# crowsonkb/style_transfer2

Hardware: AMD Instinct MI355X
Metric: style-transfer iters/sec @1024px VGG19 (higher is better)
Workload: dtype f32; 1 GPU; configs[1]: 1024x1024 single image per GPU, VGG19 to conv5_1, content conv4_2 + 5 style layers, adam fp32, 500 iterations per image; jobs=1, parallelism=independent jobs, 1 per GPU, no collective (replicas)

## Files before the change

style_transfer2_amd/csrc/gram.hip:

```cpp
#include "st2_kernels.h"
#include "env.h"
#include "wave_reduce.h"
#include <stdint.h>
#include <stdlib.h>

namespace st2 {

typedef float f32x16 __attribute__((ext_vector_type(16)));

constexpr int GKT = 32;
constexpr int GLD = GKT + 1;

GramPlan gram_plan(int C, int hw)
{
    GramPlan p;
    p.bt = C > 64 ? 128 : 64;
    const int t = (C + p.bt - 1) / p.bt;
    p.tiles = t * (t + 1) / 2;
    const int target128 = (int)env_int("ST2_GRAM_BLOCKS", 512), target64 = (int)env_int("ST2_GRAM_BLOCKS64", 1024);
    int want = p.bt == 128 ? target128 / p.tiles : (target64 + p.tiles - 1) / p.tiles;
    const int max_splits = (hw + 4 * GKT - 1) / (4 * GKT);
    if (want > max_splits) want = max_splits;
    if (want < 1) want = 1;
    int kslab = (hw + want - 1) / want;
    kslab = (kslab + GKT - 1) / GKT * GKT;
    p.kslab = kslab;
    p.splits = (hw + kslab - 1) / kslab;
    p.slab_floats = (size_t)p.splits * C * C;
    return p;
}

GramPlan gram_plan16(int C, int hw)
{
    GramPlan p = gram_plan(C, hw);
    p.kslab = (p.kslab + 63) / 64 * 64;
    p.splits = (hw + p.kslab - 1) / p.kslab;
    p.slab_floats = (size_t)p.splits * C * C;
    return p;
}

template <int BT>
__global__ __launch_bounds__(256) void gram_partial_k(const float* __restrict__ F, float* __restrict__ slabs,
                                                      int C, int hw, int tiles_1d, int kslab, GramRoi roi)
{
    constexpr int T = BT / 64;
    constexpr int ROWS_PER_T = BT / 8;
    __shared__ float As[BT * GLD];
    __shared__ float Bs[BT * GLD];

    const int tid = threadIdx.x, lane = tid & 63, wave = tid >> 6;
    const int wm = wave >> 1, wn = wave & 1;
    const int n_ut = tiles_1d * (tiles_1d + 1) / 2;
    int tile = blockIdx.x % n_ut;
    const int split = blockIdx.x / n_ut;
    int ti = 0;
    while (tile >= tiles_1d - ti) { tile -= tiles_1d - ti; ++ti; }
    const int tj = ti + tile;
    const int i0 = ti * BT, j0 = tj * BT;
    const bool diag = ti == tj;
    const int kbeg = split * kslab;
    const int kend = min(hw, kbeg + kslab);

    const int sk = tid & 31, sr = tid >> 5;
    float ra[ROWS_PER_T], rb[ROWS_PER_T];

    auto load = [&](int k0) {
        const int k = k0 + sk;
        const int ky = k / roi.rw, kx = k - ky * roi.rw;
        const size_t pix = (size_t)(roi.y0 + ky) * roi.pitch + roi.x0 + kx;
#pragma unroll
        for (int it = 0; it < ROWS_PER_T; ++it) {
            const int r = sr + it * 8;
            ra[it] = (i0 + r < C && k < kend) ? F[(size_t)(i0 + r) * roi.plane + pix] : 0.f;
            if (!diag) rb[it] = (j0 + r < C && k < kend) ? F[(size_t)(j0 + r) * roi.plane + pix] : 0.f;
        }
    };
    auto store = [&]() {
#pragma unroll
        for (int it = 0; it < ROWS_PER_T; ++it) {
            const int r = sr + it * 8;
            As[r * GLD + sk] = ra[it];
            if (!diag) Bs[r * GLD + sk] = rb[it];
        }
    };

    f32x16 acc[T][T];
#pragma unroll
    for (int i = 0; i < T; ++i)
#pragma unroll
        for (int j = 0; j < T; ++j)
#pragma unroll
            for (int e = 0; e < 16; ++e) acc[i][j][e] = 0.f;

    const float* bsrc = diag ? As : Bs;
    const int khalf = lane >> 5, l31 = lane & 31;
    const float* a_base = As + (wm * (T * 32) + l31) * GLD + khalf;
    const float* b_base = bsrc + (wn * (T * 32) + l31) * GLD + khalf;

    load(kbeg);
    for (int k0 = kbeg; k0 < kend; k0 += GKT) {
        __syncthreads();
        store();
        __syncthreads();
        if (k0 + GKT < kend) load(k0 + GKT);
#pragma unroll
        for (int ks = 0; ks < GKT / 2; ++ks) {
            float av[T], bv[T];
#pragma unroll
            for (int i = 0; i < T; ++i) av[i] = a_base[i * 32 * GLD + 2 * ks];
#pragma unroll
            for (int j = 0; j < T; ++j) bv[j] = b_base[j * 32 * GLD + 2 * ks];
#pragma unroll
            for (int i = 0; i < T; ++i)
#pragma unroll
                for (int j = 0; j < T; ++j)
                    acc[i][j] = __builtin_amdgcn_mfma_f32_32x32x2f32(av[i], bv[j], acc[i][j], 0, 0, 0);
        }
    }

    float* dst = slabs + (size_t)split * C * C;
#pragma unroll
    for (int i = 0; i < T; ++i)
#pragma unroll
        for (int j = 0; j < T; ++j) {
            const int col = j0 + wn * (T * 32) + j * 32 + l31;
#pragma unroll
            for (int e = 0; e < 16; ++e) {
                const int row = i0 + wm * (T * 32) + i * 32 + (e & 3) + 8 * (e >> 2) + 4 * khalf;
                if (row < C && col < C) dst[(size_t)row * C + col] = acc[i][j][e];
            }
        }
}

typedef __attribute__((address_space(3))) void* gram_lptr_t;
typedef float gf32x4 __attribute__((ext_vector_type(4)));

template <int BT>
__device__ __forceinline__ void gram_partial_dma_body(const float* __restrict__ F, unsigned f_bytes, float* __restrict__ slabs,
                                                      int C, int hw, int tiles_1d, int kslab)
{
    constexpr int T = BT / 64;
    constexpr int IMG = BT * 32;
    constexpr int PIECES = IMG / 256;
    constexpr int PPW = PIECES / 4;
    __shared__ __attribute__((aligned(16))) float smem[2][2][IMG];

    const int tid = threadIdx.x, lane = tid & 63;
    const int wave = __builtin_amdgcn_readfirstlane(tid >> 6);
    const int wm = wave >> 1, wn = wave & 1;
    const int n_ut = tiles_1d * (tiles_1d + 1) / 2;
    int tile = blockIdx.x % n_ut;
    const int split = blockIdx.x / n_ut;
    int ti = 0;
    while (tile >= tiles_1d - ti) { tile -= tiles_1d - ti; ++ti; }
    const int tj = ti + tile;
    const int i0 = ti * BT, j0 = tj * BT;
    const bool diag = ti == tj;
    const int kbeg = split * kslab;
    const int kend = min(hw, kbeg + kslab);
    const int nsteps = (kend - kbeg) / 32;

    const __amdgpu_buffer_rsrc_t rs = __builtin_amdgcn_make_buffer_rsrc((void*)F, 0, f_bytes, 0x00020000);
    unsigned aoff[PPW], boff[PPW];
#pragma unroll
    for (int t = 0; t < PPW; ++t) {
        const int slot = (wave + 4 * t) * 64 + lane;
        const int r = slot >> 3, q = (slot & 7) ^ ((r >> 1) & 7);
        aoff[t] = i0 + r < C ? ((unsigned)(i0 + r) * (unsigned)hw + (unsigned)kbeg + 4u * q) * 4u : 0xffffffffu;
        boff[t] = j0 + r < C ? ((unsigned)(j0 + r) * (unsigned)hw + (unsigned)kbeg + 4u * q) * 4u : 0xffffffffu;
    }
    auto dma = [&](int step, int stage) {
        const unsigned so = (unsigned)step * 128u;
#pragma unroll
        for (int t = 0; t < PPW; ++t) {
            __builtin_amdgcn_raw_ptr_buffer_load_lds(rs, (gram_lptr_t)(smem[stage][0] + (wave + 4 * t) * 256), 16,
                                                     aoff[t] == 0xffffffffu ? aoff[t] : aoff[t] + so, 0, 0, 0);
            if (!diag)
                __builtin_amdgcn_raw_ptr_buffer_load_lds(rs, (gram_lptr_t)(smem[stage][1] + (wave + 4 * t) * 256), 16,
                                                         boff[t] == 0xffffffffu ? boff[t] : boff[t] + so, 0, 0, 0);
        }
    };

    f32x16 acc[T][T];
#pragma unroll
    for (int i = 0; i < T; ++i)
#pragma unroll
        for (int j = 0; j < T; ++j)
#pragma unroll
            for (int e = 0; e < 16; ++e) acc[i][j][e] = 0.f;

    const int l31 = lane & 31;
    const bool hi = lane >= 32;
    int arow[T], brow[T];
#pragma unroll
    for (int i = 0; i < T; ++i) { arow[i] = wm * (T * 32) + i * 32 + l31; brow[i] = wn * (T * 32) + i * 32 + l31; }

    if (nsteps > 0) dma(0, 0);
    for (int st = 0; st < nsteps; ++st) {
        const int cur = st & 1;
        asm volatile("s_waitcnt vmcnt(0)" ::: "memory");
        __syncthreads();
        if (st + 1 < nsteps) dma(st + 1, cur ^ 1);
        const float* As = smem[cur][0];
        const float* Bs = diag ? smem[cur][0] : smem[cur][1];
#pragma unroll
        for (int q = 0; q < 8; ++q) {
            float a0[T], a1[T], b0[T], b1[T];
#pragma unroll
            for (int i = 0; i < T; ++i) {
                const gf32x4 v = *reinterpret_cast<const gf32x4*>(As + (arow[i] * 8 + (q ^ ((arow[i] >> 1) & 7))) * 4);
                a0[i] = hi ? v.y : v.x; a1[i] = hi ? v.w : v.z;
            }
#pragma unroll
            for (int j = 0; j < T; ++j) {
                const gf32x4 v = *reinterpret_cast<const gf32x4*>(Bs + (brow[j] * 8 + (q ^ ((brow[j] >> 1) & 7))) * 4);
                b0[j] = hi ? v.y : v.x; b1[j] = hi ? v.w : v.z;
            }
#pragma unroll
            for (int i = 0; i < T; ++i)
#pragma unroll
                for (int j = 0; j < T; ++j) {
                    acc[i][j] = __builtin_amdgcn_mfma_f32_32x32x2f32(a0[i], b0[j], acc[i][j], 0, 0, 0);
                    acc[i][j] = __builtin_amdgcn_mfma_f32_32x32x2f32(a1[i], b1[j], acc[i][j], 0, 0, 0);
                }
        }
    }

    const int khalf = lane >> 5;
    float* dst = slabs + (size_t)split * C * C;
#pragma unroll
    for (int i = 0; i < T; ++i)
#pragma unroll
        for (int j = 0; j < T; ++j) {
            const int col = j0 + wn * (T * 32) + j * 32 + l31;
#pragma unroll
            for (int e = 0; e < 16; ++e) {
                const int row = i0 + wm * (T * 32) + i * 32 + (e & 3) + 8 * (e >> 2) + 4 * khalf;
                if (row < C && col < C) dst[(size_t)row * C + col] = acc[i][j][e];
            }
        }
}

__global__ __launch_bounds__(256, 2) void gram_partial_dma_128(const float* F, unsigned f_bytes, float* slabs, int C, int hw, int tiles_1d, int kslab)
{ gram_partial_dma_body<128>(F, f_bytes, slabs, C, hw, tiles_1d, kslab); }
__global__ __launch_bounds__(256, 2) void gram_partial_dma_64(const float* F, unsigned f_bytes, float* slabs, int C, int hw, int tiles_1d, int kslab)
{ gram_partial_dma_body<64>(F, f_bytes, slabs, C, hw, tiles_1d, kslab); }

hipError_t launch_gram_partial(const float* F, float* slabs, int C, int hw, const GramPlan& pl, hipStream_t s,
                               const GramRoi* roi_in)
{
    const int t1 = (C + pl.bt - 1) / pl.bt;
    const unsigned grid = (unsigned)(pl.tiles * pl.splits);
    GramRoi roi = roi_in ? *roi_in : GramRoi{0, 0, hw, hw, (size_t)hw};
    if (!roi_in && !env_off("ST2_GRAM_DMA") && hw % 32 == 0 && pl.kslab % 32 == 0 && (reinterpret_cast<uintptr_t>(F) & 15) == 0 &&
        4ull * C * hw < 0xfffffff0ull) {
        const unsigned fb = (unsigned)(4ull * C * hw);
        if (pl.bt == 128) gram_partial_dma_128<<<grid, 256, 0, s>>>(F, fb, slabs, C, hw, t1, pl.kslab);
        else gram_partial_dma_64<<<grid, 256, 0, s>>>(F, fb, slabs, C, hw, t1, pl.kslab);
        return hipGetLastError();
    }
    if (pl.bt == 128) gram_partial_k<128><<<grid, 256, 0, s>>>(F, slabs, C, hw, t1, pl.kslab, roi);
    else gram_partial_k<64><<<grid, 256, 0, s>>>(F, slabs, C, hw, t1, pl.kslab, roi);
    return hipGetLastError();
}

__global__ __launch_bounds__(256) void gram_reduce_k(const float* __restrict__ slabs, const float* __restrict__ target,
                                                     float* __restrict__ out, float* __restrict__ partial,
                                                     int cc, int splits, float n, int C, int out_ld, int bt)
{
    __shared__ float scratch[4];
    float acc[1] = {0.f};
    for (int i = blockIdx.x * 256 + threadIdx.x; i < cc; i += gridDim.x * 256) {
        const int r = i / C, c = i - r * C;
        const int tr = r / bt, tc = c / bt;
        if (tr > tc) continue;
        float sum = 0.f;
        for (int s = 0; s < splits; ++s) sum += slabs[(size_t)s * cc + i];
        float v = sum / n;
        if (target) v -= target[i];
        out[r * out_ld + c] = v;
        acc[0] += v * v;
        if (tr < tc) { out[c * out_ld + r] = v; acc[0] += v * v; }
    }
    block_sum(acc, scratch);
    if (threadIdx.x == 0 && partial) partial[blockIdx.x] = acc[0];
}

__global__ __launch_bounds__(256) void gram_fold_k(const float* __restrict__ slabs, float* __restrict__ folded,
                                                   int cc, int splits, int per_group, int C, int bt)
{
    const int i = blockIdx.x * 256 + threadIdx.x;
    const int g = blockIdx.y;
    if (i >= cc) return;
    if ((i / C) / bt > (i % C) / bt) return;
    const int s0 = g * per_group, s1 = min(splits, s0 + per_group);
    float sum = 0.f;
    for (int s = s0; s < s1; ++s) sum += slabs[(size_t)s * cc + i];
    folded[(size_t)g * cc + i] = sum;
}

template <int GR_LANES>
__global__ __launch_bounds__(256) void gram_reduce_wide_k(const float* __restrict__ slabs, const float* __restrict__ target,
                                                          float* __restrict__ out, float* __restrict__ partial,
                                                          int cc, int splits, float n, int C, int out_ld, int bt)
{
    constexpr int GR_QUADS = 256 / GR_LANES, GR_ELEMS = 4 * GR_QUADS;
    __shared__ float4 part_s[GR_LANES][GR_QUADS];
    __shared__ float scratch[4];
    const int q = threadIdx.x % GR_QUADS, ln = threadIdx.x / GR_QUADS;
    float acc[1] = {0.f};
    for (int base = blockIdx.x * GR_ELEMS; base < cc; base += gridDim.x * GR_ELEMS) {
        const int i = base + 4 * q;
        const int r = i < cc ? i / C : 0, c = i < cc ? i - r * C : 0;
        const bool live = i < cc && r / bt <= c / bt;
        float4 sum = make_float4(0.f, 0.f, 0.f, 0.f);
        if (live)
            for (int s = ln; s < splits; s += GR_LANES) {
                const float4 v = *reinterpret_cast<const float4*>(slabs + (size_t)s * cc + i);
                sum.x += v.x; sum.y += v.y; sum.z += v.z; sum.w += v.w;
            }
        __syncthreads();
        part_s[ln][q] = sum;
        __syncthreads();
        if (ln == 0 && live) {
            float4 tot = part_s[0][q];
#pragma unroll
            for (int j = 1; j < GR_LANES; ++j) { const float4 p = part_s[j][q]; tot.x += p.x; tot.y += p.y; tot.z += p.z; tot.w += p.w; }
            float v[4] = {tot.x / n, tot.y / n, tot.z / n, tot.w / n};
            if (target) { const float4 t = *reinterpret_cast<const float4*>(target + i); v[0] -= t.x; v[1] -= t.y; v[2] -= t.z; v[3] -= t.w; }
            const bool mirror = r / bt < c / bt;
#pragma unroll
            for (int k = 0; k < 4; ++k) {
                out[r * out_ld + c + k] = v[k];
                acc[0] += v[k] * v[k];
                if (mirror) { out[(c + k) * out_ld + r] = v[k]; acc[0] += v[k] * v[k]; }
            }
        }
    }
    block_sum(acc, scratch);
    if (threadIdx.x == 0 && partial) partial[blockIdx.x] = acc[0];
}

int gram_fold_groups(const GramPlan& pl) { return pl.splits > 32 ? 32 : 0; }

hipError_t launch_gram_reduce(const float* slabs, float* folded, const float* target, float* out, int out_ld, float* partial,
                              int* n_partial, int C, double divisor, const GramPlan& pl, hipStream_t s)
{
    const int cc = C * C;
    int splits = pl.splits;
    if (splits > 32 && C % 4 == 0 && pl.bt % 4 == 0 && env_int("ST2_GRAM_REDUCE", 1) != 2) {
        const bool small = cc <= 128 * 128;
        const int grid = reduce_grid((size_t)cc, small ? 32 : 128, kMaxPartials);
        if (n_partial) *n_partial = grid;
        if (small) gram_reduce_wide_k<32><<<grid, 256, 0, s>>>(slabs, target, out, partial, cc, splits, (float)divisor, C, out_ld, pl.bt);
        else gram_reduce_wide_k<8><<<grid, 256, 0, s>>>(slabs, target, out, partial, cc, splits, (float)divisor, C, out_ld, pl.bt);
        return hipGetLastError();
    }
    const int groups = gram_fold_groups(pl);
    if (groups) {
        const int per = (pl.splits + groups - 1) / groups;
        gram_fold_k<<<dim3((cc + 255) / 256, groups), 256, 0, s>>>(slabs, folded, cc, pl.splits, per, C, pl.bt);
        slabs = folded;
        splits = (pl.splits + per - 1) / per;
    }
    const int grid = reduce_grid((size_t)cc, 256, kMaxPartials);
    if (n_partial) *n_partial = grid;
    gram_reduce_k<<<grid, 256, 0, s>>>(slabs, target, out, partial, cc, splits, (float)divisor, C, out_ld, pl.bt);
    return hipGetLastError();
}

}
```

Measured before the change: 142.2 it/s.

## Add 4-stage DMA ring gram kernel for single-tile 64-channel layers

```diff
diff --git a/style_transfer2_amd/csrc/gram.hip b/style_transfer2_amd/csrc/gram.hip
--- a/style_transfer2_amd/csrc/gram.hip
+++ b/style_transfer2_amd/csrc/gram.hip
@@ -246,6 +246,114 @@
 __global__ __launch_bounds__(256, 2) void gram_partial_dma_64(const float* F, unsigned f_bytes, float* slabs, int C, int hw, int tiles_1d, int kslab)
 { gram_partial_dma_body<64>(F, f_bytes, slabs, C, hw, tiles_1d, kslab); }
 
+constexpr int GR_STAGES = 4;
+
+__global__ __launch_bounds__(256, 2) void gram_partial_dma_64_ring(const float* F, unsigned f_bytes, float* slabs, int C, int hw, int kslab)
+{
+    constexpr int IMG = 64 * 32;
+    __shared__ __attribute__((aligned(16))) float smem[GR_STAGES][IMG];
+
+    const int tid = threadIdx.x, lane = tid & 63;
+    const int wave = __builtin_amdgcn_readfirstlane(tid >> 6);
+    const int split = blockIdx.x;
+    const int kbeg = split * kslab;
+    const int kend = min(hw, kbeg + kslab);
+    const int nsteps = (kend - kbeg) / 32;
+
+    const __amdgpu_buffer_rsrc_t rs = __builtin_amdgcn_make_buffer_rsrc((void*)F, 0, f_bytes, 0x00020000);
+    unsigned aoff[2];
+#pragma unroll
+    for (int t = 0; t < 2; ++t) {
+        const int slot = (wave + 4 * t) * 64 + lane;
+        const int r = slot >> 3, q = (slot & 7) ^ ((r >> 1) & 7);
+        aoff[t] = r < C ? ((unsigned)r * (unsigned)hw + (unsigned)kbeg + 4u * q) * 4u : 0xffffffffu;
+    }
+    auto dma = [&](int step) {
+        const unsigned so = (unsigned)step * 128u;
+        float* stage = smem[step & (GR_STAGES - 1)];
+#pragma unroll
+        for (int t = 0; t < 2; ++t)
+            __builtin_amdgcn_raw_ptr_buffer_load_lds(rs, (gram_lptr_t)(stage + (wave + 4 * t) * 256), 16,
+                                                     aoff[t] == 0xffffffffu ? aoff[t] : aoff[t] + so, 0, 0, 0);
+    };
+
+    f32x16 acc00, acc01, acc11;
+#pragma unroll
+    for (int e = 0; e < 16; ++e) { acc00[e] = 0.f; acc01[e] = 0.f; acc11[e] = 0.f; }
+
+    const int l31 = lane & 31, khalf = lane >> 5;
+    const bool hi = lane >= 32;
+    const int key = (l31 >> 1) & 7;
+
+#pragma unroll
+    for (int st = 0; st < GR_STAGES - 1; ++st)
+        if (st < nsteps) dma(st);
+    for (int st = 0; st < nsteps; ++st) {
+        const int later = min(nsteps - 1 - st, GR_STAGES - 2);
+        if (later == 2) asm volatile("s_waitcnt vmcnt(4) lgkmcnt(0)\n\ts_barrier" ::: "memory");
+        else if (later == 1) asm volatile("s_waitcnt vmcnt(2) lgkmcnt(0)\n\ts_barrier" ::: "memory");
+        else asm volatile("s_waitcnt vmcnt(0) lgkmcnt(0)\n\ts_barrier" ::: "memory");
+        if (st + GR_STAGES - 1 < nsteps) dma(st + GR_STAGES - 1);
+        const float* As = smem[st & (GR_STAGES - 1)];
+#pragma unroll
+        for (int qq = 0; qq < 2; ++qq) {
+            const int q = 2 * wave + qq;
+            const gf32x4 v0 = *reinterpret_cast<const gf32x4*>(As + (l31 * 8 + (q ^ key)) * 4);
+            const gf32x4 v1 = *reinterpret_cast<const gf32x4*>(As + ((32 + l31) * 8 + (q ^ key)) * 4);
+            const float a0 = hi ? v0.y : v0.x, a1 = hi ? v0.w : v0.z;
+            const float b0 = hi ? v1.y : v1.x, b1 = hi ? v1.w : v1.z;
+            acc00 = __builtin_amdgcn_mfma_f32_32x32x2f32(a0, a0, acc00, 0, 0, 0);
+            acc01 = __builtin_amdgcn_mfma_f32_32x32x2f32(a0, b0, acc01, 0, 0, 0);
+            acc11 = __builtin_amdgcn_mfma_f32_32x32x2f32(b0, b0, acc11, 0, 0, 0);
+            acc00 = __builtin_amdgcn_mfma_f32_32x32x2f32(a1, a1, acc00, 0, 0, 0);
+            acc01 = __builtin_amdgcn_mfma_f32_32x32x2f32(a1, b1, acc01, 0, 0, 0);
+            acc11 = __builtin_amdgcn_mfma_f32_32x32x2f32(b1, b1, acc11, 0, 0, 0);
+        }
+    }
+
+    float* red = &smem[0][0];
+    auto park = [&](int slot, const f32x16& a) {
+#pragma unroll
+        for (int e = 0; e < 16; ++e) {
+            const int row = (e & 3) + 8 * (e >> 2) + 4 * khalf;
+            red[slot * 1024 + row * 32 + (l31 ^ row)] = a[e];
+        }
+    };
+    auto total = [&](int first, int stride, int row, int col) {
+        const int at = row * 32 + (col ^ row);
+        float s = red[first * 1024 + at];
+#pragma unroll
+        for (int w = 1; w < 4; ++w) s += red[(first + w * stride) * 1024 + at];
+        return s;
+    };
+    float* dst = slabs + (size_t)split * C * C;
+    __syncthreads();
+    park(2 * wave, acc00);
+    park(2 * wave + 1, acc01);
+    __syncthreads();
+#pragma unroll
+    for (int i = 0; i < 8; ++i) {
+        const int el = tid + 256 * i, blk = el >> 10, r = (el >> 5) & 31, c = el & 31;
+        const float s = total(blk, 2, r, c);
+        if (r < C && 32 * blk + c < C) dst[(size_t)r * C + 32 * blk + c] = s;
+    }
+#pragma unroll
+    for (int i = 0; i < 4; ++i) {
+        const int el = tid + 256 * i, r = el >> 5, c = el & 31;
+        const float s = total(1, 2, c, r);
+        if (32 + r < C) dst[(size_t)(32 + r) * C + c] = s;
+    }
+    __syncthreads();
+    park(wave, acc11);
+    __syncthreads();
+#pragma unroll
+    for (int i = 0; i < 4; ++i) {
+        const int el = tid + 256 * i, r = el >> 5, c = el & 31;
+        const float s = total(0, 1, r, c);
+        if (32 + r < C && 32 + c < C) dst[(size_t)(32 + r) * C + 32 + c] = s;
+    }
+}
+
 hipError_t launch_gram_partial(const float* F, float* slabs, int C, int hw, const GramPlan& pl, hipStream_t s,
                                const GramRoi* roi_in)
 {
@@ -256,6 +364,7 @@
         4ull * C * hw < 0xfffffff0ull) {
         const unsigned fb = (unsigned)(4ull * C * hw);
         if (pl.bt == 128) gram_partial_dma_128<<<grid, 256, 0, s>>>(F, fb, slabs, C, hw, t1, pl.kslab);
+        else if (t1 == 1 && !env_off("ST2_GRAM_DMA_RING")) gram_partial_dma_64_ring<<<grid, 256, 0, s>>>(F, fb, slabs, C, hw, pl.kslab);
         else gram_partial_dma_64<<<grid, 256, 0, s>>>(F, fb, slabs, C, hw, t1, pl.kslab);
         return hipGetLastError();
     }
```

After: 142.5 it/s, median of 6. No clear change (+0.2%).
